# hamaadshah/gan_deeplearning4j

Hardware: NVIDIA H100
Metric: images/sec (full G+D step) (higher is better)
Workload: dtype bf16

## Files before the change

gan_deeplearning4j_b200/_lib.py:

```python
from __future__ import annotations

import ctypes as C
import os

_HERE = os.path.dirname(os.path.abspath(__file__))
LIB_PATH = os.path.join(_HERE, "lib", "libb200gan.so")
NAME_LEN = 64


class B200GanError(RuntimeError):
    def __init__(self, code, msg):
        super().__init__(f"libb200gan error {code}: {msg}")
        self.code = code


class LayerDesc(C.Structure):
    _fields_ = [("type", C.c_int32), ("name", C.c_char * NAME_LEN), ("n_in", C.c_int32), ("n_out", C.c_int32),
                ("k_h", C.c_int32), ("k_w", C.c_int32), ("s_h", C.c_int32), ("s_w", C.c_int32), ("p_h", C.c_int32), ("p_w", C.c_int32),
                ("has_bias", C.c_int32), ("act", C.c_int32), ("act_alpha", C.c_float), ("updater", C.c_int32),
                ("lr", C.c_float), ("beta1", C.c_float), ("beta2", C.c_float), ("eps", C.c_float), ("l2", C.c_float),
                ("bn_decay", C.c_float), ("bn_eps", C.c_float), ("pre_h", C.c_int32), ("pre_w", C.c_int32), ("pre_c", C.c_int32),
                ("loss", C.c_int32), ("frozen", C.c_int32)]


# ... 17 lines not shown
                ("a", C.c_float), ("b", C.c_float), ("additive", C.c_int32)]


class Constraint(C.Structure):
    _fields_ = [("kind", C.c_int32), ("dims_mask", C.c_int32), ("max_norm", C.c_double), ("min_norm", C.c_double), ("rate", C.c_double)]


class ConvGeom(C.Structure):
    _fields_ = [(k, C.c_int32) for k in ("n", "h", "w", "c", "oh", "ow", "o", "kh", "kw", "sh", "sw", "ph", "pw")]


class TestConvOpts(C.Structure):
    _fields_ = [("epi", C.c_int32), ("act", C.c_int32), ("alpha", C.c_float), ("bias", C.POINTER(C.c_float)), ("scale", C.POINTER(C.c_float)),
                ("groups", C.c_int32), ("aux", C.POINTER(C.c_float)), ("aux2", C.POINTER(C.c_float)), ("stats", C.POINTER(C.c_double)), ("kernel", C.c_char * 64),
                ("bn", C.c_int32), ("max_ctas", C.c_int32), ("poison", C.c_int32), ("w_mn", C.c_int32), ("per_tap", C.c_int32), ("slab", C.c_int32),
                ("defer", C.c_int32), ("db", C.POINTER(C.c_float)), ("param_offset", C.c_int32), ("splits", C.c_int32)]


class EwReduceJob(C.Structure):
    _fields_ = [("n", C.c_int64), ("stride", C.c_int64), ("src_off", C.c_int64), ("dst_off", C.c_int64), ("splits", C.c_int32), ("wide", C.c_int32)]


class TestEwOpts(C.Structure):
    _fields_ = [("op", C.c_int32), ("n", C.c_int64), ("rows", C.c_int32), ("cols", C.c_int32), ("groups", C.c_int32), ("splits", C.c_int32),
                ("stride", C.c_int64)] + [(k, C.c_int32) for k in ("N", "H", "W", "C", "KH", "KW", "SH", "SW", "act")] + [
                ("alpha", C.c_float), ("clip_eps", C.c_float), ("offset", C.c_int32), ("in_place", C.c_int32), ("accumulate", C.c_int32),
                ("poison", C.c_int32), ("n_jobs", C.c_int32), ("jobs", C.POINTER(EwReduceJob)), ("n_seg", C.c_int32),
                ("seg_off", C.POINTER(C.c_int64)), ("seg_len", C.POINTER(C.c_int64)), ("seg_coef", C.POINTER(C.c_float)), ("sumsq", C.c_double),
                ("kernel", C.c_char * 64), ("loss", C.c_int32)]


# ... 103 lines not shown
```

gan_deeplearning4j_b200/csrc/engine.cu:

```cuda
#include <cuda_runtime.h>
#include <dlfcn.h>
#include <math.h>
#include <stdarg.h>
#include <stdio.h>
#include <stdlib.h>
#include <string.h>

#include <algorithm>
#include <string>
#include <vector>

#include "../../include/b200gan.h"
#include "kernels.h"

using namespace b2g;

static thread_local char g_err[1024] = "";
static int32_t fail(int32_t code, const char* fmt, ...) {
  va_list ap; va_start(ap, fmt); vsnprintf(g_err, sizeof(g_err), fmt, ap); va_end(ap); return code;
}
#define CU(call) do { cudaError_t e_ = (call); if (e_ != cudaSuccess) return fail(B2G_ERR_CUDA, "%s:%d %s -> %s", __FILE__, __LINE__, #call, cudaGetErrorString(e_)); } while (0)
#define B2(call) do { int32_t r_ = (call); if (r_ != 0) return r_; } while (0)
#define CHECK_KERNELS() CU(cudaGetLastError())

// ... 1755 lines not shown
    if (!h || prec == PREC_F32) return downF(h, (const float*)d, count);
    float* f = nullptr; B2(upF(nullptr, count, &f)); k_nhwc_to_nchw_f32(prec, d, f, 1, 1, (int)count, s); return downF(h, f, count); }
  int32_t event(cudaEvent_t* e) { CU(cudaEventCreate(e)); events.push_back(*e); return 0; }
};
}

extern "C" int32_t b2g_ctx_allreduce_test(b2g_ctx* c, float* host, int64_t n) {
  if (!c || !host || n < 1) return fail(B2G_ERR_ARG, "null"); if (!c->comm) return fail(B2G_ERR_NCCL, "no communicator"); CU(cudaSetDevice(c->device));
  HookMem m(c->stream, PREC_F32); float* d = nullptr;
  B2(m.upF(host, (size_t)n, &d));
  NC(g_nccl.ar(d, d, (size_t)n, 7, 0, c->comm, c->stream));
  B2(m.downF(host, d, (size_t)n)); CU(cudaStreamSynchronize(c->stream)); return 0;
}

struct TcTestSchedule {
  TcTestSchedule(int bn, int max_ctas, int per_tap, int splits) { g_tc_test_bn = bn; g_tc_test_max_ctas = max_ctas; g_tc_test_per_tap = per_tap; g_tc_test_splits = splits; }
  ~TcTestSchedule() { reset(); }
  void reset() { g_tc_test_bn = 0; g_tc_test_max_ctas = 0; g_tc_test_per_tap = 0; g_tc_test_splits = 0; }
};
enum : unsigned { CO_STATS = 1u << EPI_STATS, CO_BNBWD = 1u << EPI_BNBWD, CO_ACTBWD = 1u << EPI_ACTBWD, CO_BIAS_ACT = 1u << 4, CO_SCALE = 1u << 5,
                  CO_POFF = 1u << 6, CO_BN = 1u << 7, CO_MAX_CTAS = 1u << 8, CO_PER_TAP = 1u << 9, CO_W_MN = 1u << 10, CO_SPLITS = 1u << 11,
                  CO_DEFER = 1u << 12, CO_DB = 1u << 13 };
struct ConvHookImpl {
  const char* kernel;
  bool bf16, tma;
  struct { bool (*shape)(const ConvGeom&); unsigned opts; } kind[3];
};
static bool any_shape(const ConvGeom&) { return true; }
static bool dense_bwd_shape(const ConvGeom& g) { return dense_small_o_supported(g) || dense_small_k_supported(g); }
static bool tc_edge_conv_shape(const ConvGeom& g) { return edge_conv_small_cin_supported(g) && tc_edge_conv_supported(g); }
static bool tc_edge_wgrad_shape(const ConvGeom& g) { return edge_wgrad_small_cin_supported(g) && tc_edge_wgrad_supported(g); }
static const unsigned CO_TC = CO_STATS | CO_BNBWD | CO_ACTBWD | CO_BIAS_ACT | CO_SCALE | CO_BN | CO_MAX_CTAS | CO_PER_TAP;
static const ConvHookImpl kConvHook[6] = {
  {"SIMT kernel", false, false, {{any_shape, CO_BIAS_ACT | CO_SCALE | CO_POFF}, {any_shape, CO_BIAS_ACT | CO_SCALE | CO_POFF}, {any_shape, CO_POFF}}},
  {"tensor-core kernel (BF16, a working tensor-map encoder)", true, true,
   {{tc_fprop_supported, CO_TC | CO_W_MN}, {tc_dgrad_supported, CO_TC}, {tc_wgrad_supported, CO_POFF | CO_SPLITS | CO_DEFER}}},
  {"skinny-layer kernel (<= 4 image channels)", false, false,
   {{edge_conv_small_cin_supported, CO_BIAS_ACT | CO_POFF}, {edge_deconv_small_c_supported, CO_BIAS_ACT | CO_POFF}, {edge_wgrad_small_cin_supported, CO_POFF}}},
  {"skinny-layer tensor-core kernel (BF16, <= 4 image channels, a working tensor-map encoder)", true, true,
   {{tc_edge_conv_shape, CO_BIAS_ACT | CO_MAX_CTAS}, {tc_deconv_ps_supported, CO_ACTBWD | CO_BIAS_ACT | CO_MAX_CTAS},
    {tc_edge_wgrad_shape, CO_POFF | CO_SPLITS | CO_DEFER | CO_DB}}},
  {"dense kernel (1x1 geometry: <= 4 output units, or a short reduction in the input / weight gradient)", false, false,
   {{dense_small_o_supported, CO_BIAS_ACT | CO_POFF}, {dense_bwd_shape, CO_BIAS_ACT | CO_POFF}, {dense_bwd_shape, CO_POFF}}},
  {"few-output conv kernel (BF16, O <= 4, C % 8 == 0, k x k)", true, false,
   {{head_conv_supported, CO_BIAS_ACT | CO_POFF}, {head_conv_supported, CO_BIAS_ACT | CO_POFF}, {head_conv_supported, CO_POFF | CO_SPLITS | CO_DB}}},
};
static constexpr int ik(int impl, int kind) { return 3 * impl + kind; }

extern "C" int32_t b2g_test_conv_ex(b2g_ctx* c, int32_t kind, int32_t impl, int32_t precision, const b2g_conv_geom* gg, const float* a_host, const float* b_host, float* out, int32_t iters, float* ms_per_iter,
                                    b2g_test_conv_opts* opt) {
  if (!c || !gg || !a_host || !b_host || !out) return fail(B2G_ERR_ARG, "null");
// ... 9 lines not shown
    return fail(B2G_ERR_UNSUPPORTED, "impl %d kind %d: no %s for this shape", impl, kind, im.kernel);
  const b2g_test_conv_opts none{}; const b2g_test_conv_opts& o = opt ? *opt : none;
  const struct { unsigned flag; bool set; const char* what; } asked[] = {
    {o.epi >= EPI_STATS && o.epi <= EPI_ACTBWD ? 1u << o.epi : 1u, o.epi != 0,
     "fused epilogue (epi 1-3: the tensor-core fprop / dgrad, impl 1 kind 0 / 1; epi 3: the pixel-shuffle deconv, impl 3 kind 1)"},
    {CO_BIAS_ACT, o.bias || o.act, "bias / activation (kinds 0 / 1; impl 4 kind 1 on its short-reduction kernel)"},
    {CO_SCALE, o.scale != nullptr, "scale (the SIMT and tensor-core fprop / dgrad, impl 0 / 1 kind 0 / 1)"},
    {CO_POFF, o.param_offset != 0, "param_offset (impl 0 / 2 / 4 / 5, and the tensor-core weight gradients, impl 1 / 3 kind 2)"},
    {CO_BN, o.bn != 0, "bn (the tile width of the tensor-core fprop / dgrad, impl 1 kind 0 / 1)"},
    {CO_MAX_CTAS, o.max_ctas != 0, "max_ctas (a grid cap of tc_conv_kernel and tc_edge_conv_kernel launches, impl 1 / 3 kind 0 / 1)"},
    {CO_PER_TAP, o.per_tap != 0, "per_tap (the tensor-core fprop / dgrad, impl 1 kind 0 / 1)"},
    {CO_W_MN, o.w_mn != 0, "w_mn (the [C][O] weight operand of the 1x1 tensor-core fprop, impl 1 kind 0)"},
    {CO_SPLITS, o.splits != 0, "splits (a forced split count of the weight gradients of impl 1 / 3 / 5)"},
    {CO_DEFER, o.defer != 0, "defer (the tensor-core weight gradients, impl 1 / 3 kind 2)"},
    {CO_DB, o.db != nullptr, "db (the bias column of the edge tensor-core and few-output weight gradients, impl 3 / 5 kind 2)"},
  };
  for (const auto& a : asked) if (a.set && !(im.kind[kind].opts & a.flag)) return fail(B2G_ERR_UNSUPPORTED, "impl %d kind %d takes no %s", impl, kind, a.what);
  if (o.param_offset < 0 || o.max_ctas < 0 || o.splits < 0)
    return fail(B2G_ERR_UNSUPPORTED, "param_offset %d, max_ctas %d, splits %d: none may be negative", o.param_offset, o.max_ctas, o.splits);
  if (o.bn && ((o.bn != 64 && o.bn != 128) || oc % o.bn))
    return fail(B2G_ERR_UNSUPPORTED, "bn %d: the tensor-core fprop / dgrad tile is 64 or 128 columns and must divide the %d output channels", o.bn, oc);
  if (impl == 4 && kind == 1 && (o.bias || o.act) && !dense_small_k_supported(g))
    return fail(B2G_ERR_UNSUPPORTED, "impl 4 kind 1: bias / activation run on the short-reduction kernel only, which has no variant for this shape");
  if (o.w_mn && (g.KH != 1 || g.KW != 1)) return fail(B2G_ERR_UNSUPPORTED, "w_mn: the [C][O] weight operand exists for the 1x1 tensor-core fprop only");
  const bool gemm = impl == 0 || impl == 2 || impl >= 4, tc_wg = kind == 2 && (impl == 1 || impl == 3);
  const int force_splits = o.splits;
  size_t sc = std::max(std::max(std::max(k_simt_wgrad_scratch_floats(g), k_tc_wgrad_scratch_floats(g)), std::max(k_edge_wgrad_scratch_floats(g), k_tc_edge_wgrad_scratch_floats(g))), k_dense_small_o_wgrad_scratch_floats(g)) + 16;
  if (force_splits) sc = std::max(sc, (size_t)force_splits * (impl == 1 || impl == 5 ? nw : (size_t)64 * 16 * g.C + 64) + 16);
  if (impl == 5) sc = std::max(sc, std::max(k_head_wgrad_scratch_floats(g), k_colsum_scratch_floats(g.O)) + 16);
  const size_t woff = (prec == PREC_F32 && kind != 2) ? (size_t)o.param_offset : 0, dwoff = kind == 2 ? (size_t)o.param_offset : 0;
  HookMem m(s, prec);
  float *fa, *fb, *fres, *scratch, *dbres = nullptr, *bias = nullptr, *scale = nullptr; void *ta, *tb, *to; __nv_bfloat16* wps = nullptr;
  B2(m.upF(a_host, na, &fa)); B2(m.upF(b_host, nb, &fb)); B2(m.upF(nullptr, no, &fres, dwoff)); B2(m.upF(nullptr, sc, &scratch));
  B2(m.dev(na, ts, &ta)); B2(m.dev(nb, ts, &tb, woff)); B2(m.dev(no, ts, &to)); B2(m.toT(fa, ta, na)); B2(m.toT(fb, tb, nb));
// ... 6 lines not shown
  epi.mode = o.epi; epi.scale = scale; epi.imgs_per_group = g.N / groups; epi.act = act; epi.alpha = alpha;
  if (o.epi == EPI_STATS || o.epi == EPI_BNBWD) { B2(m.dev(k_bn_acc_elems(oc, groups), 8, (void**)&d_acc)); epi.acc = d_acc; }
  if (o.epi == EPI_BNBWD || o.epi == EPI_ACTBWD) {
    if (!o.aux) return fail(B2G_ERR_ARG, "epilogue %d needs aux", o.epi);
    void* aux = nullptr; B2(m.upT(o.aux, no, &aux)); epi.aux = (const __nv_bfloat16*)aux;
  }
  if (o.epi == EPI_BNBWD) {
    if (!o.aux2) return fail(B2G_ERR_ARG, "epilogue 2 needs aux2 (the BatchNorm input z)");
    void* aux2 = nullptr; B2(m.upT(o.aux2, no, &aux2)); epi.aux2 = (const __nv_bfloat16*)aux2;
  }
  const TcEpi* pe = o.epi || o.scale ? &epi : nullptr;
  const __nv_bfloat16 *ba = (const __nv_bfloat16*)ta, *bb = (const __nv_bfloat16*)tb; __nv_bfloat16* bo = (__nv_bfloat16*)to;
  ReduceList rl{}; ReduceList* prl = o.defer ? &rl : nullptr;
  cudaEvent_t e0, e1; B2(m.event(&e0)); B2(m.event(&e1));
  int reps = iters < 1 ? 1 : iters; int rc = 0, db_written = 0;
  g_tc_last_kernel = ""; g_tc_last_slab = false; g_tc_last_splits = 0; g_gemm_last_kernel = ""; g_gemm_last_splits = 0;
  TcTestSchedule schedule(o.bn, o.max_ctas, o.per_tap != 0, force_splits);
  for (int it = -1; it < reps; ++it) {
    if (it == 0) CU(cudaEventRecord(e0, s));
    if (d_acc) CU(cudaMemsetAsync(d_acc, 0, 8 * k_bn_acc_elems(oc, groups), s));
    if (o.poison) CU(cudaMemsetAsync(to, 0xFF, ts * no, s));
    if (o.poison && kind == 2) { CU(cudaMemsetAsync(fres, 0xFF, 4 * no, s)); CU(cudaMemsetAsync(scratch, 0xFF, 4 * sc, s)); }
    if (o.poison && dbres) CU(cudaMemsetAsync(dbres, 0xFF, 4 * (size_t)g.O, s));
    switch (ik(impl, kind)) {
      case ik(0, 0): k_simt_fprop(prec, prec, g, ta, tb, bias, to, act, alpha, s, scale); break;
      case ik(0, 1): k_simt_dgrad(prec, prec, g, ta, tb, bias, to, act, alpha, s, scale); break;
      case ik(0, 2): k_simt_wgrad(prec, g, ta, tb, fres, scratch, sc, 0, s); break;
      case ik(1, 0): rc = k_tc_fprop(g, ba, bb, bias, bo, act, alpha, s, pe, o.w_mn ? 1 : 0); break;
      case ik(1, 1): rc = k_tc_dgrad(g, ba, bb, bias, bo, act, alpha, s, pe); break;
      case ik(1, 2): rc = k_tc_wgrad(g, ba, bb, fres, scratch, sc, 0, s, prl); break;
      case ik(2, 0): k_edge_conv_small_cin(prec, prec, g, ta, tb, bias, to, act, alpha, s); break;
      case ik(2, 1): k_edge_deconv_small_c(prec, prec, g, ta, tb, bias, to, act, alpha, s); break;
// ... 15 lines not shown
        const int hs = g_gemm_last_splits; k_reduce_multi(hl, s); g_gemm_last_splits = hs;
        if (dbres) { k_colsum(PREC_BF16, tb, g.N * g.OH * g.OW, g.O, scratch, dbres, 0, s); db_written = 1; }
        break;
      }
    }
    if (rc) break;
    if (o.defer) {
      if (!rl.count) { rc = -4; break; }
      k_reduce_multi(rl, s); rl.count = 0;
    }
  }
  schedule.reset();
  CU(cudaEventRecord(e1, s));
  if (rc == -4) return fail(B2G_ERR_CUDA, "defer: the weight gradient queued no reduction");
  if (rc == -5) return fail(B2G_ERR_ARG, "splits %d: the partials do not fit the scratch", force_splits);
  if (rc) return fail(B2G_ERR_CUDA, "tensor-core kernel launch failed (%d)", rc);
  if (opt) {
    strncpy(opt->kernel, gemm ? g_gemm_last_kernel : g_tc_last_kernel, sizeof(opt->kernel) - 1); opt->kernel[sizeof(opt->kernel) - 1] = 0; opt->slab = g_tc_last_slab;
    opt->splits = gemm ? g_gemm_last_splits : tc_wg ? g_tc_last_splits : 0;
  }
  if (o.db) {
    if (!db_written) return fail(B2G_ERR_UNSUPPORTED, "the edge weight gradient produces no bias column for C = %d", g.C);
    B2(m.downF(o.db, dbres, g.O));
  }
  B2(kind == 2 ? m.downF(out, fres, no) : m.downT(out, to, no));
  CU(cudaStreamSynchronize(s)); CHECK_KERNELS();
  if (d_acc && o.stats) {
    std::vector<long long> h(k_bn_acc_elems(oc, groups)); CU(cudaMemcpy(h.data(), d_acc, 8 * h.size(), cudaMemcpyDeviceToHost));
    for (int gi = 0; gi < groups; ++gi) for (int st = 0; st < 2; ++st) for (int ch = 0; ch < oc; ++ch)
      o.stats[((size_t)gi * 2 + st) * oc + ch] = (double)h[((size_t)(gi * 2 + st) * 2 + 0) * oc + ch] / 1024.0 + (double)h[((size_t)(gi * 2 + st) * 2 + 1) * oc + ch] / 1152921504606846976.0;
  }
  float ms = 0.f; CU(cudaEventElapsedTime(&ms, e0, e1)); if (ms_per_iter) *ms_per_iter = ms / reps;
  return 0;
}
// ... 445 lines not shown
```

gan_deeplearning4j_b200/csrc/kernels.h:

```cpp
#pragma once
#include <cuda_runtime.h>
#include <cuda_bf16.h>
#include <math.h>
#include <stdint.h>

namespace b2g {

enum Prec { PREC_F32 = 0, PREC_BF16 = 1 };
enum Act { ACT_IDENTITY = 0, ACT_TANH = 1, ACT_SIGMOID = 2, ACT_RELU = 3, ACT_LRELU = 4,
           ACT_ELU = 5, ACT_SELU = 6, ACT_SOFTPLUS = 7, ACT_SOFTSIGN = 8, ACT_HARDTANH = 9, ACT_HARDSIGMOID = 10, ACT_RELU6 = 11, ACT_SWISH = 12,
           ACT_CUBE = 13, ACT_RATIONALTANH = 14, ACT_RECTIFIEDTANH = 15, ACT_THRESHOLDEDRELU = 16, ACT_EXT_FIRST = ACT_ELU, ACT_EXT_LAST = ACT_THRESHOLDEDRELU };
enum Loss { LOSS_MSE = 2, LOSS_L1 = 3, LOSS_L2 = 4, LOSS_MAE = 5, LOSS_HINGE = 6, LOSS_SQUARED_HINGE = 7, LOSS_WASSERSTEIN = 8 };

inline size_t prec_size(int prec) { return prec == PREC_F32 ? 4 : 2; }

struct ConvGeom {
  int N, H, W, C;
  int OH, OW, O;
  int KH, KW, SH, SW, PH, PW;
};

extern uint64_t g_launch_count;
extern const char* g_ew_last_kernel;
int device_sm_count();
// ... 213 lines not shown
size_t k_head_wgrad_scratch_floats(const ConvGeom& g);
void k_head_fwd(const ConvGeom& g, const __nv_bfloat16* x, const __nv_bfloat16* w, const float* bias, __nv_bfloat16* out, int act, float alpha, cudaStream_t s);
void k_head_dgrad(const ConvGeom& g, const __nv_bfloat16* dy, const __nv_bfloat16* w, const float* bias, __nv_bfloat16* dx, int act, float alpha, cudaStream_t s);
int k_head_wgrad(const ConvGeom& g, const __nv_bfloat16* x, const __nv_bfloat16* dy, float* dw, float* part, size_t part_floats, int force_splits, cudaStream_t s,
                 ReduceList* defer);

bool tc_fprop_supported(const ConvGeom& g);
bool tc_dgrad_supported(const ConvGeom& g);
bool tc_wgrad_supported(const ConvGeom& g);
int  tc_init();
extern const char* g_tc_last_kernel;
extern int g_tc_test_bn, g_tc_test_max_ctas;
extern int g_tc_test_per_tap;
extern bool g_tc_last_slab;
extern int g_tc_test_splits, g_tc_last_splits;
enum { EPI_PLAIN = 0, EPI_STATS = 1, EPI_BNBWD = 2, EPI_ACTBWD = 3 };
struct TcEpi {
  int mode;
  const float* scale;
  unsigned long long* acc;
  int imgs_per_group;
  const __nv_bfloat16* aux;
  const __nv_bfloat16* aux2;
  int act; float alpha;
};
int k_tc_fprop(const ConvGeom& g, const __nv_bfloat16* x, const __nv_bfloat16* w, const float* bias, __nv_bfloat16* out, int act, float alpha, cudaStream_t s, const TcEpi* epi = nullptr, int w_mn = 0);
int k_tc_dgrad(const ConvGeom& g, const __nv_bfloat16* dy, const __nv_bfloat16* w, const float* bias, __nv_bfloat16* dx, int act, float alpha, cudaStream_t s, const TcEpi* epi = nullptr);
int k_tc_wgrad(const ConvGeom& g, const __nv_bfloat16* x, const __nv_bfloat16* dy, float* dw, float* scratch, size_t scratch_floats, int accumulate, cudaStream_t s, ReduceList* defer = nullptr);
size_t k_tc_wgrad_scratch_floats(const ConvGeom& g);
bool tc_deconv_ps_shape(const ConvGeom& g);
// ... 12 lines not shown
```

gan_deeplearning4j_b200/csrc/kernels_tc.cu:

```cuda
#include <cuda.h>
#include <stdio.h>
#include <stdlib.h>
#include <algorithm>

#include "common.cuh"
#include "kernels.h"

namespace b2g {

typedef CUresult (*PFN_encodeTiled)(CUtensorMap*, CUtensorMapDataType, cuuint32_t, void*, const cuuint64_t*, const cuuint64_t*, const cuuint32_t*,
                                    const cuuint32_t*, CUtensorMapInterleave, CUtensorMapSwizzle, CUtensorMapL2promotion, CUtensorMapFloatOOBfill);
static PFN_encodeTiled g_encode = nullptr;

int tc_init() {
  if (g_encode) return 0;
  void* fn = nullptr; cudaDriverEntryPointQueryResult q;
  if (cudaGetDriverEntryPoint("cuTensorMapEncodeTiled", &fn, cudaEnableDefault, &q) != cudaSuccess || !fn || q != cudaDriverEntryPointSuccess) return -1;
  g_encode = (PFN_encodeTiled)fn; return 0;
}

static int make_map_bf16(CUtensorMap* m, const void* base, int rank, const cuuint64_t* dims, const cuuint64_t* strides_bytes, const cuuint32_t* box, const cuuint32_t* estr) {
  if (!g_encode) return -1;
  CUresult r = g_encode(m, CU_TENSOR_MAP_DATA_TYPE_BFLOAT16, (cuuint32_t)rank, const_cast<void*>(base), dims, strides_bytes, box, estr, CU_TENSOR_MAP_INTERLEAVE_NONE,
                        CU_TENSOR_MAP_SWIZZLE_128B, CU_TENSOR_MAP_L2_PROMOTION_L2_256B, CU_TENSOR_MAP_FLOAT_OOB_FILL_NONE);
// ... 21 lines not shown
}
__device__ __forceinline__ void tma_load_3d(uint32_t dst, const CUtensorMap* map, uint32_t bar, int c0, int c1, int c2) {
  asm volatile("cp.async.bulk.tensor.3d.shared::cluster.global.tile.mbarrier::complete_tx::bytes [%0], [%1, {%3, %4, %5}], [%2];"
               ::"r"(dst), "l"(map), "r"(bar), "r"(c0), "r"(c1), "r"(c2) : "memory");
}
__device__ __forceinline__ void tma_load_2d(uint32_t dst, const CUtensorMap* map, uint32_t bar, int c0, int c1) {
  asm volatile("cp.async.bulk.tensor.2d.shared::cluster.global.tile.mbarrier::complete_tx::bytes [%0], [%1, {%3, %4}], [%2];"
               ::"r"(dst), "l"(map), "r"(bar), "r"(c0), "r"(c1) : "memory");
}
__device__ __forceinline__ bool elect_one_sync() {
  uint32_t pred = 0;
  asm volatile("{\n\t.reg .pred P1;\n\t.reg .b32 rx;\n\telect.sync rx|P1, %1;\n\t@P1 mov.s32 %0, 1;\n\t}" : "+r"(pred) : "r"(0xffffffffu));
  return pred != 0;
}
__device__ __forceinline__ void prefetch_map(const CUtensorMap* map) { asm volatile("prefetch.tensormap [%0];" ::"l"(map) : "memory"); }
__device__ __forceinline__ void fence_proxy_async_smem() { asm volatile("fence.proxy.async.shared::cta;" ::: "memory"); }

__device__ __forceinline__ uint64_t gmma_desc(uint32_t saddr, uint32_t lbo_bytes) {
  return (uint64_t)((saddr & 0x3FFFFu) >> 4) | ((uint64_t)((lbo_bytes >> 4) & 0x3FFF) << 16) | ((uint64_t)(1024 >> 4) << 32) | (1ull << 62);
}
__device__ __forceinline__ uint64_t desc_kmajor_sw128(uint32_t saddr) { return gmma_desc(saddr, 16); }
__device__ __forceinline__ uint64_t desc_mnmajor_sw128(uint32_t saddr, uint32_t lbo_bytes) { return gmma_desc(saddr, lbo_bytes); }

__device__ __forceinline__ void wg_fence() { asm volatile("wgmma.fence.sync.aligned;" ::: "memory"); }
__device__ __forceinline__ void wg_commit() { asm volatile("wgmma.commit_group.sync.aligned;" ::: "memory"); }
template <int N>
__device__ __forceinline__ void wg_wait() { asm volatile("wgmma.wait_group.sync.aligned %0;" ::"n"(N) : "memory"); }

template <int TA, int TB>
__device__ __forceinline__ void wgmma_n64(float (&d)[32], uint64_t da, uint64_t db) {
// ... 404 lines not shown
        const int group = p.imgs_per_group > 0 ? n0 / p.imgs_per_group : 0;
        epi_tile<BN, EPI, AFFINE>(p, srow, pix * p.OC + nb0, nb0, group, sst, reinterpret_cast<uint4*>(smem_gen + S::STG_OFF) + ew * 128, q, lane,
                                  (int)threadIdx.x - 256, half * (BN / 2), (half + 1) * (BN / 2));
        if constexpr (EPI == EPI_STATS || EPI == EPI_BNBWD) epi_bar_sync();
      }
      mbar_arrive(park_empty + 8 * k);
      if (++k == S::PARKS) { k = 0; kph ^= 1; }
    }
  }
}

const char* g_tc_last_kernel = "";
bool g_tc_last_slab = false;
int g_tc_test_bn = 0, g_tc_test_max_ctas = 0, g_tc_test_per_tap = 0, g_tc_test_splits = 0;
int g_tc_last_splits = 0;
static int tc_device() { int dev = 0; cudaGetDevice(&dev); return dev < 0 || dev >= 64 ? 0 : dev; }
#define TC_SET_SMEM_ONCE(kernel, bytes)                                                                                            \
  do { static bool set_[64] = {}; const int d_ = tc_device();                                                                       \
       if (!set_[d_]) { if (cudaFuncSetAttribute(kernel, cudaFuncAttributeMaxDynamicSharedMemorySize, (int)(bytes)) != cudaSuccess) return -2; set_[d_] = true; } } while (0)

static bool pick_row_tile(int N, int GH, int GW, int rows, int* Nt, int* Ht, int* Wt) {
  const int P = GH * GW;
  if (GW > rows || rows % GW) return false;
  if (P >= rows) { if (P % rows) return false; *Nt = 1; *Ht = rows / GW; *Wt = GW; return GH % *Ht == 0; }
  if (rows % P || N % (rows / P)) return false;
  *Nt = rows / P; *Ht = GH; *Wt = GW; return true;
}
static int pick_bn(int OC) { return OC % 128 == 0 ? 128 : OC % 64 == 0 ? 64 : 0; }
static int pick_bn_fill(int OC, long m_tiles_x_phases) {
  if (g_tc_test_bn) return g_tc_test_bn;
// ... 374 lines not shown
  int KW, SH, SW, PH, PW;
  int taps, C;
  int kb_total, kb_per_split;
  float* out; size_t split_stride;
};

template <int BNW, int STAGES>
struct TcWgradSmem {
  static constexpr int A_BYTES = 2 * 64 * 128;
  static constexpr int B_BYTES = (BNW / 64) * 64 * 128;
  static constexpr int STAGE_BYTES = A_BYTES + B_BYTES;
  static constexpr int BAR_OFF = STAGES * STAGE_BYTES;
  static constexpr int TOTAL = BAR_OFF + 256 + 1024;
};

template <int BNW, int STAGES>
__global__ void __launch_bounds__(TC_THREADS, 1) tc_wgrad_kernel(const __grid_constant__ CUtensorMap tmDy, const __grid_constant__ CUtensorMap tmX, const TcWgradParams p) {
  using S = TcWgradSmem<BNW, STAGES>;
  constexpr int NB = BNW / 64;
  extern __shared__ uint8_t smem_raw[];
  const uint32_t smem_base = (smem_u32(smem_raw) + 1023u) & ~1023u;
  const uint32_t bar_full = smem_base + S::BAR_OFF, bar_empty = bar_full + 8 * STAGES;
  const int warp = threadIdx.x >> 5, lane = threadIdx.x & 31;
  const int split = blockIdx.x, col0 = blockIdx.y * BNW, o0 = blockIdx.z * 128;
  const int kb_beg = split * p.kb_per_split, kb_end = min(p.kb_total, kb_beg + p.kb_per_split);
  const int num_kb = max(0, kb_end - kb_beg);

  if (threadIdx.x == 0) {
    prefetch_map(&tmDy); prefetch_map(&tmX);
    for (int s = 0; s < STAGES; ++s) { mbar_init(bar_full + 8 * s, 1); mbar_init(bar_empty + 8 * s, 8); }
    fence_mbar_init();
  }
  __syncthreads();
  pdl_trigger();
  pdl_wait();

  if (warp == 0) {
    int xc[NB], xw[NB], xh[NB];
#pragma unroll
    for (int j = 0; j < NB; ++j) { const int col = col0 + j * 64, tap = col / p.C; xc[j] = col % p.C; xw[j] = -p.PW + tap % p.KW; xh[j] = -p.PH + tap / p.KW; }
    int n0, y0;
    if (p.Nt > 1) { n0 = kb_beg * p.Nt; y0 = 0; } else { n0 = kb_beg / p.tiles_y; y0 = (kb_beg % p.tiles_y) * p.Ht; }
    int s = 0; uint32_t ph = 0;
    for (int i = 0; i < num_kb; ++i) {
      const int kb = kb_beg + i;
      mbar_wait(bar_empty + 8 * s, ph ^ 1);
      if (elect_one_sync()) {
        mbar_expect_tx(bar_full + 8 * s, S::STAGE_BYTES);
        const uint32_t a = smem_base + s * S::STAGE_BYTES, b = a + S::A_BYTES;
        tma_load_2d(a, &tmDy, bar_full + 8 * s, o0, kb * 64);
        tma_load_2d(a + 8192, &tmDy, bar_full + 8 * s, o0 + 64, kb * 64);
#pragma unroll
        for (int j = 0; j < NB; ++j) tma_load_4d(b + j * 8192, &tmX, bar_full + 8 * s, xc[j], xw[j], y0 * p.SH + xh[j], n0);
      }
      __syncwarp();
      if (++s == STAGES) { s = 0; ph ^= 1; }
      if (p.Nt > 1) n0 += p.Nt; else { y0 += p.Ht; if (y0 >= p.tiles_y * p.Ht) { y0 = 0; ++n0; } }
    }
  } else if (warp >= 4) {
    const int wg = (warp >> 2) - 1;
    float acc[NB][32];
#pragma unroll
    for (int nb = 0; nb < NB; ++nb)
#pragma unroll
      for (int j = 0; j < 32; ++j) acc[nb][j] = 0.f;
    int s = 0, prev = -1; uint32_t ph = 0;
    for (int i = 0; i < num_kb; ++i) {
      mbar_wait(bar_full + 8 * s, ph);
      wg_fence();
      const uint32_t a = smem_base + s * S::STAGE_BYTES + wg * 8192, b = smem_base + s * S::STAGE_BYTES + S::A_BYTES;
#pragma unroll
      for (int k = 0; k < 4; ++k) {
        if constexpr (NB == 2) wgmma_n128<1, 1>(acc[0], acc[1], desc_mnmajor_sw128(a + k * 2048, 8192), desc_mnmajor_sw128(b + k * 2048, 8192));
        else wgmma_n64<1, 1>(acc[0], desc_mnmajor_sw128(a + k * 2048, 8192), desc_mnmajor_sw128(b + k * 2048, 8192));
      }
      wg_commit();
      wg_wait<1>();
      if (prev >= 0 && lane == 0) mbar_arrive(bar_empty + 8 * prev);
      prev = s;
      if (++s == STAGES) { s = 0; ph ^= 1; }
    }
    wg_wait<0>();
#pragma unroll
    for (int i = 0; i < 2; ++i) {
      const int o = o0 + wg * 64 + (warp & 3) * 16 + (lane >> 2) + 8 * i;
      float* orow = p.out + (size_t)split * p.split_stride + (size_t)o * p.taps * p.C + col0;
#pragma unroll
      for (int nb = 0; nb < NB; ++nb)
#pragma unroll
        for (int j = 0; j < 8; ++j)
          *reinterpret_cast<float2*>(orow + nb * 64 + j * 8 + 2 * (lane & 3)) = make_float2(acc[nb][4 * j + 2 * i], acc[nb][4 * j + 2 * i + 1]);
    }
  }
}

static int wgrad_bnw(const ConvGeom& g) { if (g.C % 64) return 0; const long cols = (long)g.KH * g.KW * g.C; return cols % 128 == 0 ? 128 : 64; }
static int wgrad_target() { return (2 * device_sm_count()) / 3; }
static int wgrad_splits_for(const ConvGeom& g, int o_tile) {
  const int bnw = wgrad_bnw(g); if (!bnw) return 1;
  long tiles = (long)(g.O / o_tile) * (g.KH * g.KW * g.C / bnw), kbt = (long)g.N * g.OH * g.OW / 64;
  long sp = wgrad_target() / tiles, cap = kbt / 8; if (cap < 1) cap = 1; if (sp > cap) sp = cap; if (sp < 1) sp = 1; return (int)sp;
}
static int tc_wgrad_splits(const ConvGeom& g) { return g_tc_test_splits > 0 ? g_tc_test_splits : wgrad_splits_for(g, 128); }
bool tc_wgrad_supported(const ConvGeom& g) {
  int a, b, c;
  return g.O % 128 == 0 && wgrad_bnw(g) != 0 && g.SH >= 1 && g.SH <= 2 && g.SW == g.SH && ((long)g.N * g.OH * g.OW) % 64 == 0 &&
         pick_row_tile(g.N, g.OH, g.OW, 64, &a, &b, &c) && c * g.SW <= 256 && b * g.SH <= 256;
}
size_t k_tc_wgrad_scratch_floats(const ConvGeom& g) {
  if (!tc_wgrad_supported(g)) return 0;
  return (size_t)wgrad_splits_for(g, 128) * g.O * g.KH * g.KW * g.C;
}

template <int BNW, int STAGES>
static int launch_wgrad(const CUtensorMap& tmDy, const CUtensorMap& tmX, const TcWgradParams& p, dim3 grid, cudaStream_t s, const char* name) {
  using S = TcWgradSmem<BNW, STAGES>;
  TC_SET_SMEM_ONCE((tc_wgrad_kernel<BNW, STAGES>), S::TOTAL);
  launch_pdl(tc_wgrad_kernel<BNW, STAGES>, dim3(grid), dim3(TC_THREADS), (size_t)(S::TOTAL), s, tmDy, tmX, p);
  LAUNCHED(); g_tc_last_kernel = name;
  return cudaPeekAtLastError() == cudaSuccess ? 0 : -3;
}

static void reduce_or_defer(ReduceList* defer, const float* src, float* dst, size_t n, int splits, size_t stride, int accumulate, cudaStream_t s) {
  if (defer && !accumulate && defer->count < ReduceList::MAX_JOBS) { reduce_list_push(defer, src, dst, (int64_t)n, splits, (int64_t)stride); return; }
  k_reduce_splits(src, dst, n, splits, stride, accumulate, s);
}

int k_tc_wgrad(const ConvGeom& g, const __nv_bfloat16* x, const __nv_bfloat16* dy, float* dw, float* scratch, size_t scratch_floats, int accumulate, cudaStream_t s, ReduceList* defer) {
  TcWgradParams p{};
  if (!pick_row_tile(g.N, g.OH, g.OW, 64, &p.Nt, &p.Ht, &p.Wt)) return -1;
  const int BNW = wgrad_bnw(g); const size_t n = (size_t)g.O * g.KH * g.KW * g.C;
  int splits = tc_wgrad_splits(g);
  if ((size_t)splits * n > scratch_floats) return -5;
  p.tiles_y = g.OH / p.Ht; p.KW = g.KW; p.SH = g.SH; p.SW = g.SW; p.PH = g.PH; p.PW = g.PW; p.taps = g.KH * g.KW; p.C = g.C;
// ... 20 lines not shown
```

gan_deeplearning4j_b200/engine.py:

```python
from __future__ import annotations

import copy
import ctypes as C
import math
from typing import Dict, List, Optional, Sequence

import numpy as np

from . import _lib
from ._lib import GanConfig, LayerDesc, LrSchedule, NetConfig, check

LAYER_TYPES = {"conv2d": 0, "deconv2d": 1, "batchnorm": 2, "dense": 3, "activation": 4, "maxpool": 5, "upsample2d": 6,
               "output": 7, "loss": 8, "ff_to_cnn": 9, "cnn_to_ff": 10, "dropout": 11, "subsampling": 12, "global_pooling": 13,
               "cnn_loss": 14, "elementwise": 15, "merge": 16}
ELEMENTWISE_OPS = {"add": 0, "subtract": 1, "product": 2, "average": 3, "max": 4}
VERTEX_TYPES = ("elementwise", "merge")
POOLINGS = {"max": 0, "avg": 1, "sum": 2, "pnorm": 3}
GLOBAL_PNORM_DEFAULT = 2
ACTS = {"identity": 0, "tanh": 1, "sigmoid": 2, "relu": 3, "lrelu": 4, "elu": 5, "selu": 6, "softplus": 7, "softsign": 8, "hardtanh": 9,
        "hardsigmoid": 10, "relu6": 11, "swish": 12, "cube": 13, "rationaltanh": 14, "rectifiedtanh": 15, "thresholdedrelu": 16}
ACT_ALPHA_DEFAULTS = {"elu": 1.0, "thresholdedrelu": 1.0}
LOSSES = {"xent": 0, "mcxent": 1, "mse": 2, "l1": 3, "l2": 4, "mae": 5, "hinge": 6, "squared_hinge": 7, "wasserstein": 8}
UPDATERS = {"sgd": 0, "rmsprop": 1, "adam": 2, "noop": 3, "nesterovs": 4, "adagrad": 5, "adamax": 6, "nadam": 7, "amsgrad": 8, "adadelta": 9}
NO_LR_UPDATERS = ("noop", "adadelta")
# ... 612 lines not shown
def test_conv(ctx: Context, kind: int, impl: int, precision: int, geom: Dict[str, int], a, b, out_size: int, iters: int = 1):
    g = _lib.ConvGeom(**geom)
    a, b = _f32(a).ravel(), _f32(b).ravel()
    out = np.empty(out_size, np.float32)
    ms = C.c_float()
    check(ctx.lib.b2g_test_conv(ctx.h, kind, impl, precision, C.byref(g), _fp(a), _fp(b), _fp(out), iters, C.byref(ms)))
    return out, ms.value


EPI_PLAIN, EPI_STATS, EPI_BNBWD, EPI_ACTBWD = 0, 1, 2, 3


def test_conv_ex(ctx: Context, kind: int, geom: Dict[str, int], a, b, out_size: int, *, epi: int = 0, act: str = "identity", alpha: float = 0.0,
                 bias=None, scale=None, groups: int = 1, aux=None, aux2=None, iters: int = 1, impl: int = 1, bn: int = 0, max_ctas: int = 0,
                 poison: bool = False, w_mn: bool = False, per_tap: bool = False, info: Optional[dict] = None, defer: bool = False, db=None,
                 precision: int = BF16, param_offset: int = 0, splits: int = 0):
    g = _lib.ConvGeom(**geom)
    a, b = _f32(a).ravel(), _f32(b).ravel()
    out = np.empty(out_size, np.float32)
    oc = geom["o"] if kind == 0 else geom["c"]
    o = _lib.TestConvOpts()
    o.epi, o.act, o.alpha, o.groups = epi, ACTS[act], alpha, groups
    o.bn, o.max_ctas, o.poison, o.w_mn, o.per_tap, o.defer = bn, max_ctas, int(poison), int(w_mn), int(per_tap), int(defer)
    o.param_offset, o.splits = param_offset, splits
    if db is not None:
        assert db.dtype == np.float32 and db.flags.c_contiguous
        o.db = _fp(db)
    keep = []
    for name, v in (("bias", bias), ("scale", scale), ("aux", aux), ("aux2", aux2)):
        if v is not None:
            arr = _f32(v).ravel(); keep.append(arr); setattr(o, name, _fp(arr))
    stats = None
    if epi in (EPI_STATS, EPI_BNBWD):
        stats = np.zeros((groups, 2, oc), np.float64); o.stats = stats.ctypes.data_as(C.POINTER(C.c_double))
    ms = C.c_float()
    check(ctx.lib.b2g_test_conv_ex(ctx.h, kind, impl, precision, C.byref(g), _fp(a), _fp(b), _fp(out), iters, C.byref(ms), C.byref(o)))
    if info is not None:
        info["slab"], info["splits"] = bool(o.slab), o.splits
    return out, stats, o.kernel.decode(), ms.value


def test_bn(ctx: Context, precision: int, path: int, x, eps_out, gamma, beta, run_mean, run_var, *, act: str = "identity", alpha: float = 0.0,
            eps: float = 1e-5, decay: float = 0.9, g_gamma=None, g_beta=None, want_param_grads: bool = True):
    x, e = _f32(x), _f32(eps_out)
    groups, rows, ch = x.shape
    par = [_f32(v).ravel() for v in (gamma, beta, run_mean, run_var)]
    r = {k: np.empty(x.shape, np.float32) for k in ("y", "eps_in")}
    r["g_gamma"] = _f32(np.zeros(ch) if g_gamma is None else g_gamma).copy()
    r["g_beta"] = _f32(np.zeros(ch) if g_beta is None else g_beta).copy()
    r.update({k: np.empty(ch, np.float32) for k in ("g_mean", "g_var")})
    r.update({k: np.empty((groups, ch), np.float32) for k in ("mean", "invstd")})
    check(ctx.lib.b2g_test_bn(ctx.h, precision, path, groups, rows, ch, _fp(x), _fp(e), *[_fp(v) for v in par], ACTS[act], alpha, eps, decay,
                              int(want_param_grads), *[_fp(r[k]) for k in ("y", "eps_in", "g_gamma", "g_beta", "g_mean", "g_var", "mean", "invstd")]))
# ... 64 lines not shown
```

include/b200gan.h:

```cpp
#ifndef B200GAN_H
#define B200GAN_H

#include <stddef.h>
#include <stdint.h>

#ifdef __cplusplus
extern "C" {
#endif

#define B2G_VERSION 101
#define B2G_NAME_LEN 64

typedef struct b2g_ctx b2g_ctx;
typedef struct b2g_net b2g_net;
typedef struct b2g_gan b2g_gan;

typedef enum {
  B2G_OK = 0,
  B2G_ERR_ARG = -1,
  B2G_ERR_SHAPE = -2,
  B2G_ERR_CUDA = -3,
  B2G_ERR_NCCL = -4,
  B2G_ERR_OOM = -5,
  B2G_ERR_UNSUPPORTED = -6,
// ... 191 lines not shown
  int32_t act; float alpha;
  const float* bias;
  const float* scale;
  int32_t groups;
  const float* aux;
  const float* aux2;
  double* stats;
  char kernel[64];
  int32_t bn;
  int32_t max_ctas;
  int32_t poison;
  int32_t w_mn;
  int32_t per_tap;
  int32_t slab;
  int32_t defer;
  float* db;
  int32_t param_offset;
  int32_t splits;
} b2g_test_conv_opts;
int32_t b2g_test_conv_ex(b2g_ctx* ctx, int32_t kind, int32_t impl, int32_t precision, const b2g_conv_geom* g,
                         const float* x_or_dy, const float* w_or_x, float* out, int32_t iters, float* ms_per_iter, b2g_test_conv_opts* opts);

int32_t b2g_test_hbm_kernels(b2g_net* net, int32_t rows, int32_t channels, int32_t iters, float* ms3);

int32_t b2g_test_bn(b2g_ctx* ctx, int32_t precision, int32_t path, int32_t groups, int32_t rows, int32_t C, const float* x, const float* eps_out,
                    const float* gamma, const float* beta, const float* run_mean, const float* run_var, int32_t act, float alpha, float eps, float decay,
                    int32_t want_param_grads, float* y, float* eps_in, float* g_gamma, float* g_beta, float* g_mean, float* g_var, float* mean, float* invstd);
int32_t b2g_test_net_shadow(b2g_net* net, int32_t layer, int32_t which, float* out, int64_t n);
int32_t b2g_test_net_noisy_operand(b2g_net* net, int32_t layer, int32_t which, float* out, int64_t n);
int32_t b2g_test_dropout(b2g_ctx* ctx, int32_t precision, uint64_t seed, int32_t layer, int32_t rank, int64_t pass, int32_t rows, int32_t h, int32_t w,
// ... 54 lines not shown
```

Before: 92180.

## Multicast shared wgrad operand tiles across thread-block clusters via TMA

Adds thread-block cluster variants of the tensor-core weight-gradient kernel. CTAs that share dy or x tiles along the y/z grid dimensions load them once with TMA multicast, and consumers release each stage by arriving on the empty barriers of every sharing CTA through mapa remote arrives. By default a 2-wide cluster along y is chosen when grid.z is 1 and grid.y is even. This is meant to cut duplicate global and L2 traffic for the dy operand, at the cost of cross-CTA synchronisation, cluster scheduling limits, and exit-time cluster barriers.

```diff
diff --git a/gan_deeplearning4j_b200/_lib.py b/gan_deeplearning4j_b200/_lib.py
--- a/gan_deeplearning4j_b200/_lib.py
+++ b/gan_deeplearning4j_b200/_lib.py
@@ -55,7 +55,7 @@
     _fields_ = [("epi", C.c_int32), ("act", C.c_int32), ("alpha", C.c_float), ("bias", C.POINTER(C.c_float)), ("scale", C.POINTER(C.c_float)),
                 ("groups", C.c_int32), ("aux", C.POINTER(C.c_float)), ("aux2", C.POINTER(C.c_float)), ("stats", C.POINTER(C.c_double)), ("kernel", C.c_char * 64),
                 ("bn", C.c_int32), ("max_ctas", C.c_int32), ("poison", C.c_int32), ("w_mn", C.c_int32), ("per_tap", C.c_int32), ("slab", C.c_int32),
-                ("defer", C.c_int32), ("db", C.POINTER(C.c_float)), ("param_offset", C.c_int32), ("splits", C.c_int32)]
+                ("defer", C.c_int32), ("cluster", C.c_int16 * 2), ("db", C.POINTER(C.c_float)), ("param_offset", C.c_int32), ("splits", C.c_int32)]
 
 
 class EwReduceJob(C.Structure):
diff --git a/gan_deeplearning4j_b200/csrc/engine.cu b/gan_deeplearning4j_b200/csrc/engine.cu
--- a/gan_deeplearning4j_b200/csrc/engine.cu
+++ b/gan_deeplearning4j_b200/csrc/engine.cu
@@ -1793,13 +1793,16 @@
 }
 
 struct TcTestSchedule {
-  TcTestSchedule(int bn, int max_ctas, int per_tap, int splits) { g_tc_test_bn = bn; g_tc_test_max_ctas = max_ctas; g_tc_test_per_tap = per_tap; g_tc_test_splits = splits; }
+  TcTestSchedule(int bn, int max_ctas, int per_tap, int splits, const int16_t* cluster) {
+    g_tc_test_bn = bn; g_tc_test_max_ctas = max_ctas; g_tc_test_per_tap = per_tap; g_tc_test_splits = splits;
+    g_tc_test_cluster[0] = cluster[0]; g_tc_test_cluster[1] = cluster[1];
+  }
   ~TcTestSchedule() { reset(); }
-  void reset() { g_tc_test_bn = 0; g_tc_test_max_ctas = 0; g_tc_test_per_tap = 0; g_tc_test_splits = 0; }
+  void reset() { g_tc_test_bn = 0; g_tc_test_max_ctas = 0; g_tc_test_per_tap = 0; g_tc_test_splits = 0; g_tc_test_cluster[0] = g_tc_test_cluster[1] = 0; }
 };
 enum : unsigned { CO_STATS = 1u << EPI_STATS, CO_BNBWD = 1u << EPI_BNBWD, CO_ACTBWD = 1u << EPI_ACTBWD, CO_BIAS_ACT = 1u << 4, CO_SCALE = 1u << 5,
                   CO_POFF = 1u << 6, CO_BN = 1u << 7, CO_MAX_CTAS = 1u << 8, CO_PER_TAP = 1u << 9, CO_W_MN = 1u << 10, CO_SPLITS = 1u << 11,
-                  CO_DEFER = 1u << 12, CO_DB = 1u << 13 };
+                  CO_DEFER = 1u << 12, CO_DB = 1u << 13, CO_CLUSTER = 1u << 14 };
 struct ConvHookImpl {
   const char* kernel;
   bool bf16, tma;
@@ -1813,7 +1816,7 @@
 static const ConvHookImpl kConvHook[6] = {
   {"SIMT kernel", false, false, {{any_shape, CO_BIAS_ACT | CO_SCALE | CO_POFF}, {any_shape, CO_BIAS_ACT | CO_SCALE | CO_POFF}, {any_shape, CO_POFF}}},
   {"tensor-core kernel (BF16, a working tensor-map encoder)", true, true,
-   {{tc_fprop_supported, CO_TC | CO_W_MN}, {tc_dgrad_supported, CO_TC}, {tc_wgrad_supported, CO_POFF | CO_SPLITS | CO_DEFER}}},
+   {{tc_fprop_supported, CO_TC | CO_W_MN}, {tc_dgrad_supported, CO_TC}, {tc_wgrad_supported, CO_POFF | CO_SPLITS | CO_DEFER | CO_CLUSTER}}},
   {"skinny-layer kernel (<= 4 image channels)", false, false,
    {{edge_conv_small_cin_supported, CO_BIAS_ACT | CO_POFF}, {edge_deconv_small_c_supported, CO_BIAS_ACT | CO_POFF}, {edge_wgrad_small_cin_supported, CO_POFF}}},
   {"skinny-layer tensor-core kernel (BF16, <= 4 image channels, a working tensor-map encoder)", true, true,
@@ -1853,10 +1856,13 @@
     {CO_SPLITS, o.splits != 0, "splits (a forced split count of the weight gradients of impl 1 / 3 / 5)"},
     {CO_DEFER, o.defer != 0, "defer (the tensor-core weight gradients, impl 1 / 3 kind 2)"},
     {CO_DB, o.db != nullptr, "db (the bias column of the edge tensor-core and few-output weight gradients, impl 3 / 5 kind 2)"},
+    {CO_CLUSTER, o.cluster[0] != 0 || o.cluster[1] != 0, "cluster (the thread-block cluster of the tensor-core weight gradient, impl 1 kind 2)"},
   };
   for (const auto& a : asked) if (a.set && !(im.kind[kind].opts & a.flag)) return fail(B2G_ERR_UNSUPPORTED, "impl %d kind %d takes no %s", impl, kind, a.what);
   if (o.param_offset < 0 || o.max_ctas < 0 || o.splits < 0)
     return fail(B2G_ERR_UNSUPPORTED, "param_offset %d, max_ctas %d, splits %d: none may be negative", o.param_offset, o.max_ctas, o.splits);
+  if ((o.cluster[0] || o.cluster[1]) && (o.cluster[0] < 1 || o.cluster[0] > 2 || o.cluster[1] < 1 || o.cluster[1] > 2))
+    return fail(B2G_ERR_UNSUPPORTED, "cluster (%d, %d): each of cy, cz is 1 or 2", o.cluster[0], o.cluster[1]);
   if (o.bn && ((o.bn != 64 && o.bn != 128) || oc % o.bn))
     return fail(B2G_ERR_UNSUPPORTED, "bn %d: the tensor-core fprop / dgrad tile is 64 or 128 columns and must divide the %d output channels", o.bn, oc);
   if (impl == 4 && kind == 1 && (o.bias || o.act) && !dense_small_k_supported(g))
@@ -1893,8 +1899,8 @@
   ReduceList rl{}; ReduceList* prl = o.defer ? &rl : nullptr;
   cudaEvent_t e0, e1; B2(m.event(&e0)); B2(m.event(&e1));
   int reps = iters < 1 ? 1 : iters; int rc = 0, db_written = 0;
-  g_tc_last_kernel = ""; g_tc_last_slab = false; g_tc_last_splits = 0; g_gemm_last_kernel = ""; g_gemm_last_splits = 0;
-  TcTestSchedule schedule(o.bn, o.max_ctas, o.per_tap != 0, force_splits);
+  g_tc_last_kernel = ""; g_tc_last_slab = false; g_tc_last_splits = 0; g_tc_last_cluster[0] = g_tc_last_cluster[1] = 0; g_gemm_last_kernel = ""; g_gemm_last_splits = 0;
+  TcTestSchedule schedule(o.bn, o.max_ctas, o.per_tap != 0, force_splits, o.cluster);
   for (int it = -1; it < reps; ++it) {
     if (it == 0) CU(cudaEventRecord(e0, s));
     if (d_acc) CU(cudaMemsetAsync(d_acc, 0, 8 * k_bn_acc_elems(oc, groups), s));
@@ -1940,10 +1946,12 @@
   CU(cudaEventRecord(e1, s));
   if (rc == -4) return fail(B2G_ERR_CUDA, "defer: the weight gradient queued no reduction");
   if (rc == -5) return fail(B2G_ERR_ARG, "splits %d: the partials do not fit the scratch", force_splits);
+  if (rc == -6) return fail(B2G_ERR_UNSUPPORTED, "cluster (%d, %d) does not divide tc_wgrad_kernel's grid along y / z", o.cluster[0], o.cluster[1]);
   if (rc) return fail(B2G_ERR_CUDA, "tensor-core kernel launch failed (%d)", rc);
   if (opt) {
     strncpy(opt->kernel, gemm ? g_gemm_last_kernel : g_tc_last_kernel, sizeof(opt->kernel) - 1); opt->kernel[sizeof(opt->kernel) - 1] = 0; opt->slab = g_tc_last_slab;
     opt->splits = gemm ? g_gemm_last_splits : tc_wg ? g_tc_last_splits : 0;
+    opt->cluster[0] = (int16_t)g_tc_last_cluster[0]; opt->cluster[1] = (int16_t)g_tc_last_cluster[1];
   }
   if (o.db) {
     if (!db_written) return fail(B2G_ERR_UNSUPPORTED, "the edge weight gradient produces no bias column for C = %d", g.C);
diff --git a/gan_deeplearning4j_b200/csrc/kernels.h b/gan_deeplearning4j_b200/csrc/kernels.h
--- a/gan_deeplearning4j_b200/csrc/kernels.h
+++ b/gan_deeplearning4j_b200/csrc/kernels.h
@@ -251,6 +251,7 @@
 extern int g_tc_test_per_tap;
 extern bool g_tc_last_slab;
 extern int g_tc_test_splits, g_tc_last_splits;
+extern int g_tc_test_cluster[2], g_tc_last_cluster[2];
 enum { EPI_PLAIN = 0, EPI_STATS = 1, EPI_BNBWD = 2, EPI_ACTBWD = 3 };
 struct TcEpi {
   int mode;
diff --git a/gan_deeplearning4j_b200/csrc/kernels_tc.cu b/gan_deeplearning4j_b200/csrc/kernels_tc.cu
--- a/gan_deeplearning4j_b200/csrc/kernels_tc.cu
+++ b/gan_deeplearning4j_b200/csrc/kernels_tc.cu
@@ -59,6 +59,23 @@
   return pred != 0;
 }
 __device__ __forceinline__ void prefetch_map(const CUtensorMap* map) { asm volatile("prefetch.tensormap [%0];" ::"l"(map) : "memory"); }
+
+__device__ __forceinline__ void tma_load_2d_mc(uint32_t dst, const CUtensorMap* map, uint32_t bar, int c0, int c1, uint16_t mask) {
+  asm volatile("cp.async.bulk.tensor.2d.shared::cluster.global.tile.mbarrier::complete_tx::bytes.multicast::cluster [%0], [%1, {%4, %5}], [%2], %3;"
+               ::"r"(dst), "l"(map), "r"(bar), "h"(mask), "r"(c0), "r"(c1) : "memory");
+}
+__device__ __forceinline__ void tma_load_4d_mc(uint32_t dst, const CUtensorMap* map, uint32_t bar, int c0, int c1, int c2, int c3, uint16_t mask) {
+  asm volatile("cp.async.bulk.tensor.4d.shared::cluster.global.tile.mbarrier::complete_tx::bytes.multicast::cluster [%0], [%1, {%4, %5, %6, %7}], [%2], %3;"
+               ::"r"(dst), "l"(map), "r"(bar), "h"(mask), "r"(c0), "r"(c1), "r"(c2), "r"(c3) : "memory");
+}
+__device__ __forceinline__ void mbar_arrive_cluster(uint32_t bar, uint32_t cta) {
+  asm volatile("{\n\t.reg .b32 ra;\n\tmapa.shared::cluster.u32 ra, %0, %1;\n\tmbarrier.arrive.shared::cluster.b64 _, [ra];\n\t}" ::"r"(bar), "r"(cta) : "memory");
+}
+__device__ __forceinline__ void cluster_sync() { asm volatile("barrier.cluster.arrive.relaxed.aligned;\n\tbarrier.cluster.wait.aligned;" ::: "memory"); }
+__device__ __forceinline__ uint32_t cluster_ctaid_y() { uint32_t r; asm("mov.u32 %0, %%cluster_ctaid.y;" : "=r"(r)); return r; }
+__device__ __forceinline__ uint32_t cluster_ctaid_z() { uint32_t r; asm("mov.u32 %0, %%cluster_ctaid.z;" : "=r"(r)); return r; }
+__device__ __forceinline__ uint32_t cluster_nctaid_y() { uint32_t r; asm("mov.u32 %0, %%cluster_nctaid.y;" : "=r"(r)); return r; }
+__device__ __forceinline__ uint32_t cluster_nctaid_z() { uint32_t r; asm("mov.u32 %0, %%cluster_nctaid.z;" : "=r"(r)); return r; }
 __device__ __forceinline__ void fence_proxy_async_smem() { asm volatile("fence.proxy.async.shared::cta;" ::: "memory"); }
 
 __device__ __forceinline__ uint64_t gmma_desc(uint32_t saddr, uint32_t lbo_bytes) {
@@ -493,6 +510,7 @@
 bool g_tc_last_slab = false;
 int g_tc_test_bn = 0, g_tc_test_max_ctas = 0, g_tc_test_per_tap = 0, g_tc_test_splits = 0;
 int g_tc_last_splits = 0;
+int g_tc_test_cluster[2] = {0, 0}, g_tc_last_cluster[2] = {0, 0};
 static int tc_device() { int dev = 0; cudaGetDevice(&dev); return dev < 0 || dev >= 64 ? 0 : dev; }
 #define TC_SET_SMEM_ONCE(kernel, bytes)                                                                                            \
   do { static bool set_[64] = {}; const int d_ = tc_device();                                                                       \
@@ -897,7 +915,7 @@
   static constexpr int TOTAL = BAR_OFF + 256 + 1024;
 };
 
-template <int BNW, int STAGES>
+template <int BNW, int STAGES, int CY = 1, int CZ = 1>
 __global__ void __launch_bounds__(TC_THREADS, 1) tc_wgrad_kernel(const __grid_constant__ CUtensorMap tmDy, const __grid_constant__ CUtensorMap tmX, const TcWgradParams p) {
   using S = TcWgradSmem<BNW, STAGES>;
   constexpr int NB = BNW / 64;
@@ -908,13 +926,17 @@
   const int split = blockIdx.x, col0 = blockIdx.y * BNW, o0 = blockIdx.z * 128;
   const int kb_beg = split * p.kb_per_split, kb_end = min(p.kb_total, kb_beg + p.kb_per_split);
   const int num_kb = max(0, kb_end - kb_beg);
+  constexpr bool CLUSTER = CY * CZ > 1;
+  constexpr uint32_t sharers = CY + CZ - 1;
+  const uint32_t ry = CY > 1 ? cluster_ctaid_y() : 0, rz = CZ > 1 ? cluster_ctaid_z() : 0;
 
   if (threadIdx.x == 0) {
     prefetch_map(&tmDy); prefetch_map(&tmX);
-    for (int s = 0; s < STAGES; ++s) { mbar_init(bar_full + 8 * s, 1); mbar_init(bar_empty + 8 * s, 8); }
+    for (int s = 0; s < STAGES; ++s) { mbar_init(bar_full + 8 * s, 1); mbar_init(bar_empty + 8 * s, 8 * sharers); }
     fence_mbar_init();
   }
-  __syncthreads();
+  if constexpr (CLUSTER) cluster_sync();
+  else __syncthreads();
   pdl_trigger();
   pdl_wait();
 
@@ -924,6 +946,8 @@
     for (int j = 0; j < NB; ++j) { const int col = col0 + j * 64, tap = col / p.C; xc[j] = col % p.C; xw[j] = -p.PW + tap % p.KW; xh[j] = -p.PH + tap / p.KW; }
     int n0, y0;
     if (p.Nt > 1) { n0 = kb_beg * p.Nt; y0 = 0; } else { n0 = kb_beg / p.tiles_y; y0 = (kb_beg % p.tiles_y) * p.Ht; }
+    const uint16_t dy_mask = (uint16_t)(((1u << CY) - 1) << (CY * rz));
+    const uint16_t x_mask = (uint16_t)((CZ == 2 ? 1u | (1u << CY) : 1u) << ry);
     int s = 0; uint32_t ph = 0;
     for (int i = 0; i < num_kb; ++i) {
       const int kb = kb_beg + i;
@@ -931,10 +955,18 @@
       if (elect_one_sync()) {
         mbar_expect_tx(bar_full + 8 * s, S::STAGE_BYTES);
         const uint32_t a = smem_base + s * S::STAGE_BYTES, b = a + S::A_BYTES;
-        tma_load_2d(a, &tmDy, bar_full + 8 * s, o0, kb * 64);
-        tma_load_2d(a + 8192, &tmDy, bar_full + 8 * s, o0 + 64, kb * 64);
-#pragma unroll
-        for (int j = 0; j < NB; ++j) tma_load_4d(b + j * 8192, &tmX, bar_full + 8 * s, xc[j], xw[j], y0 * p.SH + xh[j], n0);
+#pragma unroll
+        for (int j = 0; j < 2; ++j) {
+          if (j % CY != ry) continue;
+          if constexpr (CY == 1) tma_load_2d(a + j * 8192, &tmDy, bar_full + 8 * s, o0 + j * 64, kb * 64);
+          else tma_load_2d_mc(a + j * 8192, &tmDy, bar_full + 8 * s, o0 + j * 64, kb * 64, dy_mask);
+        }
+#pragma unroll
+        for (int j = 0; j < NB; ++j) {
+          if (j % CZ != rz) continue;
+          if constexpr (CZ == 1) tma_load_4d(b + j * 8192, &tmX, bar_full + 8 * s, xc[j], xw[j], y0 * p.SH + xh[j], n0);
+          else tma_load_4d_mc(b + j * 8192, &tmX, bar_full + 8 * s, xc[j], xw[j], y0 * p.SH + xh[j], n0, x_mask);
+        }
       }
       __syncwarp();
       if (++s == STAGES) { s = 0; ph ^= 1; }
@@ -947,6 +979,7 @@
     for (int nb = 0; nb < NB; ++nb)
 #pragma unroll
       for (int j = 0; j < 32; ++j) acc[nb][j] = 0.f;
+    const uint32_t rel = (lane == 1 && CY == 2) ? (1 - ry) + CY * rz : ry + CY * (1 - rz);
     int s = 0, prev = -1; uint32_t ph = 0;
     for (int i = 0; i < num_kb; ++i) {
       mbar_wait(bar_full + 8 * s, ph);
@@ -959,7 +992,10 @@
       }
       wg_commit();
       wg_wait<1>();
-      if (prev >= 0 && lane == 0) mbar_arrive(bar_empty + 8 * prev);
+      if (prev >= 0) {
+        if (lane == 0) mbar_arrive(bar_empty + 8 * prev);
+        else if (CLUSTER && lane < sharers) mbar_arrive_cluster(bar_empty + 8 * prev, rel);
+      }
       prev = s;
       if (++s == STAGES) { s = 0; ph ^= 1; }
     }
@@ -975,6 +1011,7 @@
           *reinterpret_cast<float2*>(orow + nb * 64 + j * 8 + 2 * (lane & 3)) = make_float2(acc[nb][4 * j + 2 * i], acc[nb][4 * j + 2 * i + 1]);
     }
   }
+  if constexpr (CLUSTER) cluster_sync();
 }
 
 static int wgrad_bnw(const ConvGeom& g) { if (g.C % 64) return 0; const long cols = (long)g.KH * g.KW * g.C; return cols % 128 == 0 ? 128 : 64; }
@@ -995,12 +1032,35 @@
   return (size_t)wgrad_splits_for(g, 128) * g.O * g.KH * g.KW * g.C;
 }
 
+static bool wgrad_cluster(dim3 grid, int* cy, int* cz) {
+  if (g_tc_test_cluster[0]) { *cy = g_tc_test_cluster[0]; *cz = g_tc_test_cluster[1]; }
+  else { *cy = grid.z == 1 && grid.y % 2 == 0 ? 2 : 1; *cz = 1; }
+  return grid.y % *cy == 0 && grid.z % *cz == 0;
+}
+template <int BNW, int STAGES, int CY, int CZ>
+static int launch_wgrad_cluster(const CUtensorMap& tmDy, const CUtensorMap& tmX, const TcWgradParams& p, dim3 grid, cudaStream_t s) {
+  using S = TcWgradSmem<BNW, STAGES>;
+  TC_SET_SMEM_ONCE((tc_wgrad_kernel<BNW, STAGES, CY, CZ>), S::TOTAL);
+  if constexpr (CY * CZ == 1) {
+    launch_pdl(tc_wgrad_kernel<BNW, STAGES>, grid, dim3(TC_THREADS), (size_t)(S::TOTAL), s, tmDy, tmX, p);
+  } else {
+    cudaLaunchConfig_t cfg{}; cfg.gridDim = grid; cfg.blockDim = dim3(TC_THREADS); cfg.dynamicSmemBytes = S::TOTAL; cfg.stream = s;
+    cudaLaunchAttribute at[2];
+    at[0].id = cudaLaunchAttributeProgrammaticStreamSerialization; at[0].val.programmaticStreamSerializationAllowed = 1;
+    at[1].id = cudaLaunchAttributeClusterDimension; at[1].val.clusterDim.x = 1; at[1].val.clusterDim.y = CY; at[1].val.clusterDim.z = CZ;
+    cfg.attrs = at; cfg.numAttrs = 2;
+    cudaLaunchKernelEx(&cfg, tc_wgrad_kernel<BNW, STAGES, CY, CZ>, tmDy, tmX, p);
+  }
+  return 0;
+}
 template <int BNW, int STAGES>
 static int launch_wgrad(const CUtensorMap& tmDy, const CUtensorMap& tmX, const TcWgradParams& p, dim3 grid, cudaStream_t s, const char* name) {
-  using S = TcWgradSmem<BNW, STAGES>;
-  TC_SET_SMEM_ONCE((tc_wgrad_kernel<BNW, STAGES>), S::TOTAL);
-  launch_pdl(tc_wgrad_kernel<BNW, STAGES>, dim3(grid), dim3(TC_THREADS), (size_t)(S::TOTAL), s, tmDy, tmX, p);
-  LAUNCHED(); g_tc_last_kernel = name;
+  int cy, cz;
+  if (!wgrad_cluster(grid, &cy, &cz)) return -6;
+  const int rc = cy == 1 ? (cz == 1 ? launch_wgrad_cluster<BNW, STAGES, 1, 1>(tmDy, tmX, p, grid, s) : launch_wgrad_cluster<BNW, STAGES, 1, 2>(tmDy, tmX, p, grid, s))
+                         : (cz == 1 ? launch_wgrad_cluster<BNW, STAGES, 2, 1>(tmDy, tmX, p, grid, s) : launch_wgrad_cluster<BNW, STAGES, 2, 2>(tmDy, tmX, p, grid, s));
+  if (rc) return rc;
+  LAUNCHED(); g_tc_last_kernel = name; g_tc_last_cluster[0] = cy; g_tc_last_cluster[1] = cz;
   return cudaPeekAtLastError() == cudaSuccess ? 0 : -3;
 }
 
diff --git a/gan_deeplearning4j_b200/engine.py b/gan_deeplearning4j_b200/engine.py
--- a/gan_deeplearning4j_b200/engine.py
+++ b/gan_deeplearning4j_b200/engine.py
@@ -650,7 +650,7 @@
 def test_conv_ex(ctx: Context, kind: int, geom: Dict[str, int], a, b, out_size: int, *, epi: int = 0, act: str = "identity", alpha: float = 0.0,
                  bias=None, scale=None, groups: int = 1, aux=None, aux2=None, iters: int = 1, impl: int = 1, bn: int = 0, max_ctas: int = 0,
                  poison: bool = False, w_mn: bool = False, per_tap: bool = False, info: Optional[dict] = None, defer: bool = False, db=None,
-                 precision: int = BF16, param_offset: int = 0, splits: int = 0):
+                 precision: int = BF16, param_offset: int = 0, splits: int = 0, cluster=(0, 0)):
     g = _lib.ConvGeom(**geom)
     a, b = _f32(a).ravel(), _f32(b).ravel()
     out = np.empty(out_size, np.float32)
@@ -659,6 +659,7 @@
     o.epi, o.act, o.alpha, o.groups = epi, ACTS[act], alpha, groups
     o.bn, o.max_ctas, o.poison, o.w_mn, o.per_tap, o.defer = bn, max_ctas, int(poison), int(w_mn), int(per_tap), int(defer)
     o.param_offset, o.splits = param_offset, splits
+    o.cluster[0], o.cluster[1] = cluster
     if db is not None:
         assert db.dtype == np.float32 and db.flags.c_contiguous
         o.db = _fp(db)
@@ -672,7 +673,7 @@
     ms = C.c_float()
     check(ctx.lib.b2g_test_conv_ex(ctx.h, kind, impl, precision, C.byref(g), _fp(a), _fp(b), _fp(out), iters, C.byref(ms), C.byref(o)))
     if info is not None:
-        info["slab"], info["splits"] = bool(o.slab), o.splits
+        info["slab"], info["splits"], info["cluster"] = bool(o.slab), o.splits, (o.cluster[0], o.cluster[1])
     return out, stats, o.kernel.decode(), ms.value
 
 
diff --git a/include/b200gan.h b/include/b200gan.h
--- a/include/b200gan.h
+++ b/include/b200gan.h
@@ -229,6 +229,7 @@
   int32_t per_tap;
   int32_t slab;
   int32_t defer;
+  int16_t cluster[2];
   float* db;
   int32_t param_offset;
   int32_t splits;
```

Result: no change. 92190 (median of 6 runs) (+0.0%).
